# hukaixuan19970627/yolov5_obb

Measured on AMD Instinct MI355X. Metric: val.py img/s (hot path: non_max_suppression_obb, bs16) + NMS ms/img @100k cand, DOTAv1.5 1024^2, 1/2/4/8 GPU, higher is better.
Workload: dtype f16; 1 GPU; DOTAv1.5 1024^2 bs16 (BASELINE metric; configs[1] thresholds): yolov5 OBB head output (16,64512,201) fp16, 4 distinct tensors rotated (cold: 1.66 GB working set) -> non_max_suppression_obb (conf .25, iou .45, multi_label, max_det 1500), val.py --task speed hot path = dt[2] of val.py; global_batch=16, anchors_per_image=64512, nc=16, detections_per_batch=3734, parallelism=dp1 (images sharded, no data-path collective)

## Files before the change

include/obb_hip.h:

```cpp
#ifndef OBB_HIP_H
#define OBB_HIP_H

#include <stddef.h>
#include <stdint.h>

#ifdef __cplusplus
extern "C" {
#endif

#define OBB_OK 0
#define OBB_ERR_BAD_ARG (-1)
#define OBB_ERR_WORKSPACE (-2)
#define OBB_ERR_LAUNCH (-3)
#define OBB_ERR_INTERNAL (-4)
#define OBB_ERR_NO_DEVICE (-5)

#define OBB_NMS_DROP_SMALL 1

const char* obb_version(void);
int obb_device_info(int* cu_count, int* wave_size, char* arch_name, int arch_name_len);
int obb_nms_set_max_grid(int max_workgroups);

#define OBB_PROF_STAGES 8
int obb_profile_enable(int on);
int obb_profile_collect(double* ms_sum_host, int64_t* count_host, int n_stages);



size_t obb_nms_workspace_bytes(int64_t n, int64_t nseg, int kind);

int obb_nms_rotated_f32(const float* dets5, const float* scores, int64_t n, float iou_thr, int flags, int64_t max_keep,
                        int64_t* keep_out, int64_t* num_keep, void* ws, size_t ws_bytes, void* stream);

int obb_nms_rotated_f64(const double* dets5, const double* scores, int64_t n, float iou_thr, int flags, int64_t max_keep,
                        int64_t* keep_out, int64_t* num_keep, void* ws, size_t ws_bytes, void* stream);

int obb_nms_poly_f32(const float* polys, int64_t row_stride, int64_t n, float iou_thr, int64_t max_keep, int64_t* keep_out,
                     int64_t* num_keep, void* ws, size_t ws_bytes, void* stream);

int obb_merge_nms_poly_f64(const double* dets9, int64_t n, const int32_t* order, const int32_t* seg_off, int64_t nseg,
                           double thresh, int64_t* keep_out, int64_t* num_keep, void* ws, size_t ws_bytes, void* stream);

int obb_merge_nms_poly_all_f64(const double* dets9, int64_t n, const int32_t* order, const int32_t* seg_off, int64_t nseg,
                               double thresh, int64_t* keep_out, int64_t* num_keep, void* ws, size_t ws_bytes, void* stream);
// ... 131 lines not shown
```

yolov5_obb_amd/_lib.py:

```python
import ctypes as C
import os
import threading

import torch

_HERE = os.path.dirname(os.path.abspath(__file__))
LIB_PATH = os.environ.get("OBB_HIP_LIB") or os.path.join(_HERE, "libobb_hip.so")

OBB_OK = 0
OBB_NMS_DROP_SMALL = 1
_ERR = {-1: "bad argument", -2: "workspace missing or too small", -3: "kernel launch failed",
        -4: "internal error", -5: "no usable HIP device"}

_lib = None
_lock = threading.RLock()

_vp, _i64, _i32, _f32, _sz = C.c_void_p, C.c_int64, C.c_int, C.c_float, C.c_size_t

SIGNATURES = {
    "obb_version": (C.c_char_p, []),
    "obb_device_info": (_i32, [C.POINTER(_i32), C.POINTER(_i32), C.c_char_p, _i32]),
    "obb_nms_set_max_grid": (_i32, [_i32]),
    "obb_profile_enable": (_i32, [_i32]),
    "obb_profile_collect": (_i32, [_vp, _vp, _i32]),
    "obb_nms_workspace_bytes": (_sz, [_i64, _i64, _i32]),
    "obb_nms_rotated_f32": (_i32, [_vp, _vp, _i64, _f32, _i32, _i64, _vp, _vp, _vp, _sz, _vp]),
    "obb_nms_rotated_f64": (_i32, [_vp, _vp, _i64, _f32, _i32, _i64, _vp, _vp, _vp, _sz, _vp]),
    "obb_nms_poly_f32": (_i32, [_vp, _i64, _i64, _f32, _i64, _vp, _vp, _vp, _sz, _vp]),
    "obb_merge_nms_poly_f64": (_i32, [_vp, _i64, _vp, _vp, _i64, C.c_double, _vp, _vp, _vp, _sz, _vp]),
    "obb_merge_nms_poly_all_f64": (_i32, [_vp, _i64, _vp, _vp, _i64, C.c_double, _vp, _vp, _vp, _sz, _vp]),
    "obb_merge_nms_hbb_f64": (_i32, [_vp, _i64, _i64, _vp, _vp, _i64, C.c_double, _vp, _vp, _vp, _sz, _vp]),
    "obb_task1_parse_tiles": (_i64, [_vp, _i64, _i64, _vp, _vp, _vp, _vp, _vp, _vp]),
    "obb_task1_format_rows": (_i64, [_vp, _vp, _vp, _vp, _vp, _i64, _vp, _i64]),
    "obb_task1_parse_dets": (_i64, [_vp, _i64, _i64, _vp, _vp, _vp, _vp]),
    "obb_task1_parse_gt": (_i64, [_vp, _i64, _i64, _vp, _vp, _vp, _vp]),
    "obb_eval_best_gt_f64": (_i32, [_vp, _vp, _i64, _vp, _vp, _i64, _vp, _vp, _vp]),
    "obb_nms_obb_workspace_bytes": (_sz, [_i64, _i64, _i64, _i32]),
    "obb_non_max_suppression_obb": (_i32, [_vp, _i32, _i64, _i64, _i64, _f32, _f32, _vp, _i32, _i32, _i32, _i64, _i64, _f32,
                                           _vp, _i64, _i64, _i64, _vp, _i32, _vp, _vp, _vp, _sz, _vp]),
    "obb_non_max_suppression_obb_col": (_i32, [_vp, _vp, _i32, _i64, _i64, _i64, _f32, _f32, _vp, _i32, _i32, _i32, _i64, _i64, _f32,
                                               _vp, _i64, _i64, _i64, _vp, _i32, _vp, _vp, _vp, _sz, _vp]),
    "obb_nms_obb_state_bytes": (_sz, [_i64]),
    "obb_non_max_suppression_obb_st": (_i32, [_vp, _vp, _i32, _i64, _i64, _i64, _f32, _f32, _vp, _i32, _i32, _i32, _i64, _i64, _f32,
                                              _vp, _i64, _i64, _i64, _vp, _i32, _vp, _vp, _vp, _sz, _vp, _sz, _vp]),
    "obb_non_max_suppression_obb_head": (_i32, [_i32, _vp, _i32, _i64, _i64, _i64, _vp, _vp, _vp, _vp, _f32, _f32, _vp, _i32, _i32, _i32,
# ... 214 lines not shown
```

yolov5_obb_amd/csrc/nms.hip:

```cpp
#include <hip/hip_runtime.h>
#include <cstring>
#include <stdint.h>
#include <stdlib.h>
#include <stdio.h>
#include <string.h>
#include <hip/hip_fp16.h>
#include "launch_once.h"
#include "obb_device.h"
#include "nms_core.h"
#include "nms_mk.h"
#include "obb_hip.h"
#include "psrs_sort.h"
#include "nms_small.h"
#include "segsort.h"

namespace obb {

enum { PROF_DECODE = 0, PROF_SEGSORT, PROF_PREP, PROF_STEPS, PROF_GATHER, PROF_NMS_SORT, PROF_NMS_PREP, PROF_NMS_STEPS, PROF_N };
struct ProfState {
  int on = 0;
  static constexpr int kMax = 8192;
  hipEvent_t ev0[kMax], ev1[kMax];
  int id[kMax];
  int created = 0, used = 0;
// ... 1032 lines not shown
    const int want = 2048 < ProfState::kMax ? 2048 : ProfState::kMax;
    while (g_prof.created < want) {
      if (hipEventCreate(&g_prof.ev0[g_prof.created]) != hipSuccess) return OBB_ERR_INTERNAL;
      if (hipEventCreate(&g_prof.ev1[g_prof.created]) != hipSuccess) { hipEventDestroy(g_prof.ev0[g_prof.created]); return OBB_ERR_INTERNAL; }
      g_prof.created++;
    }
  }
  return OBB_OK;
}

int obb_profile_collect(double* ms_sum, int64_t* count, int n_stages) {
  for (int i = 0; i < n_stages; i++) { ms_sum[i] = 0.0; count[i] = 0; }
  for (int k = 0; k < g_prof.used; k++) {
    float ms = 0.f;
    if (hipEventSynchronize(g_prof.ev1[k]) != hipSuccess) return OBB_ERR_INTERNAL;
    if (hipEventElapsedTime(&ms, g_prof.ev0[k], g_prof.ev1[k]) != hipSuccess) return OBB_ERR_INTERNAL;
    const int id = g_prof.id[k];
    if (id < n_stages) { ms_sum[id] += ms; count[id]++; }
  }
  g_prof.used = 0;
  return OBB_OK;
}

int obb_nms_set_max_grid(int max_workgroups) {
  g_max_grid = max_workgroups > 0 ? max_workgroups : 0;
  return OBB_OK;
}

const char* obb_version(void) { return "obb_hip 0.2 (gfx950)"; }

int obb_device_info(int* cu_count, int* wave_size, char* arch_name, int arch_name_len) {
  int dev = 0;
  if (hipGetDevice(&dev) != hipSuccess) return OBB_ERR_NO_DEVICE;
  hipDeviceProp_t p;
  if (hipGetDeviceProperties(&p, dev) != hipSuccess) return OBB_ERR_NO_DEVICE;
  if (cu_count) *cu_count = p.multiProcessorCount;
  if (wave_size) *wave_size = p.warpSize;
  if (arch_name && arch_name_len > 0) { strncpy(arch_name, p.gcnArchName, arch_name_len - 1); arch_name[arch_name_len - 1] = 0; }
  return OBB_OK;
}

}

#ifdef OBB_SMALL_TRACE
extern "C" int obb_debug_small_trace2(unsigned long long* words) {
  static unsigned long long zero2[2048 * 8];
  if (hipDeviceSynchronize() != hipSuccess) return -1;
  if (hipMemcpyFromSymbol(words, HIP_SYMBOL(obb::g_small_trace2), sizeof(obb::g_small_trace2)) != hipSuccess) return -1;
  return hipMemcpyToSymbol(HIP_SYMBOL(obb::g_small_trace2), zero2, sizeof(obb::g_small_trace2)) == hipSuccess ? 0 : -1;
}
extern "C" int obb_debug_small_trace(unsigned long long* seg_words, unsigned long long* tail_words) {
  if (hipDeviceSynchronize() != hipSuccess) return -1;
  if (hipMemcpyFromSymbol(seg_words, HIP_SYMBOL(obb::g_small_trace), sizeof(obb::g_small_trace)) != hipSuccess) return -2;
  if (hipMemcpyFromSymbol(tail_words, HIP_SYMBOL(obb::g_small_trace_tail), sizeof(obb::g_small_trace_tail)) != hipSuccess) return -3;
  static unsigned long long zero[2048 * 16];
  if (hipMemcpyToSymbol(HIP_SYMBOL(obb::g_small_trace), zero, sizeof(obb::g_small_trace)) != hipSuccess) return -4;
  if (hipMemcpyToSymbol(HIP_SYMBOL(obb::g_small_trace_tail), zero, sizeof(obb::g_small_trace_tail)) != hipSuccess) return -5;
  return 0;
}
#endif
```

yolov5_obb_amd/csrc/nms_small.h:

```cpp
#pragma once

namespace obb {

#ifdef OBB_SMALL_TRACE
__device__ unsigned long long g_small_trace[2048 * 16];
__device__ unsigned long long g_small_trace_tail[2048 * 4];
__device__ unsigned long long g_small_trace2[2048 * 8];
#define STRACE(kind, ...) do { if (threadIdx.x == 0 && blockIdx.x < 2048) { const unsigned long long v_[] = {__VA_ARGS__}; unsigned long long* o_ = g_small_trace + blockIdx.x * 16; o_[0] = (kind); for (int z_ = 0; z_ < (int)(sizeof(v_) / 8) && z_ < 15; z_++) o_[1 + z_] = v_[z_]; } } while (0)
#endif
constexpr int kSmallMax = OBB_NMS_SMALL_SEG;
constexpr int kSmallWords = kSmallMax / 64;
constexpr int kSmallThreads = 512;
constexpr int kSmallWaves = kSmallThreads / 64;

struct SmallArgs {
  const float4* rec;
  const u64* alive;
  const int* seg_begin;
  const int* seg_end;
  int* keep_cnt;
  int64_t* keep_out;
  int* too_big;
  float thr;
  int max_keep;
  const unsigned long long* keys_sorted;
  const uint32_t* vals_sorted;
  const int* mode;
  int ncs;
  unsigned long long* pub_key;
  uint32_t* pub_val;
  long long n_pos;
  int helpers;
  const int* help_cnt;
  const int* work;
  const int* seg_np;
  int* seg_ticket;
  u64* part_main;
  u64* part_help;
  const unsigned long long* keys_in;
  const float4* cand;
  const int* cnt;
  const int* tiny;
  long long cap_img, max_nms, A;
  int nc;
  float class_offset;
  int* seg_max;
};
struct SmallFromSort { static constexpr bool kSelf = false; };
constexpr int kSmallClipWaves = 4;
constexpr int kSmallSplit1 = 128;
constexpr int kSmallHelpMax = 256;
__host__ __device__ __forceinline__ int small_parts(int n) {
  return n <= kSmallSplit1 ? 1 : (n <= 192 ? 2 : (n <= 256 ? 4 : (n <= 320 ? 6 : 8)));
}
struct SmallNoTail {
  struct Args {};
  static __device__ __forceinline__ void run(const SmallArgs&, const Args&, unsigned char*, int) {}
};

template <class G>
__device__ __attribute__((noinline)) int small_quick(const float4* ra, const float4* rb, float thr) {
  return G::classify_quick(ra, rb, thr, true);
}

template <class G>
__device__ __attribute__((noinline)) uint32_t small_slice_bits(const float4* s_rec, int i0, int n, uint32_t arow16, float4 cq, int j, bool jv) {
  const int lane = threadIdx.x & 63;
  const int ir = i0 + (lane & 15);
  const float4 rq = s_rec[(ir < n ? ir : 0) * G::RECQ];
// ... 4 lines not shown
    const float dx = cq.x - a.x, dy = cq.y - a.y;
    const float rs = a.z + cq.z;
    const float d2 = dx * dx + dy * dy;
    const bool apart = (d2 > rs * rs) & (fminf(a.w, cq.w) >= 2.34e-9f * d2);
    const bool row_ok = ((arow16 >> r) & 1u) != 0u && i0 + r < n;
    const bool pass = !apart & jv & (j > i0 + r) & row_ok;
    bits |= pass ? (1u << r) : 0u;
  }
  return bits;
}

template <class G>
struct SmallWave {
  float scr[G::SCR * 64];
  uint32_t q0[128], q1[128], q2[128];
};

template <class G, class FRONT>
__device__ __forceinline__ int small_segment(const SmallArgs& a, unsigned char* s_raw) {
  __shared__ int s_next, s_nkept, s_qcnt[kSmallWaves], s_qhead[kSmallWaves], s_qcnt2[kSmallWaves], s_last;
  __shared__ uint32_t s_kept[kSmallMax];
  __shared__ unsigned long long s_pk[kSmallMax];
  __shared__ uint32_t s_pv[kSmallMax];
  float4* s_rec = reinterpret_cast<float4*>(s_raw);
  u64* s_mask = reinterpret_cast<u64*>(s_rec + (size_t)kSmallMax * G::RECQ);
  u64* s_alive = s_mask + (size_t)kSmallMax * kSmallWords;
  SmallWave<G>* s_wave = reinterpret_cast<SmallWave<G>*>(s_alive + 8);
  const int tid = threadIdx.x, lane = tid & 63, wv = tid >> 6;
  int seg = (int)blockIdx.x - a.helpers, part = 0, np = 1, hbase = 0;
  if (seg < 0) {
    const int h = (int)blockIdx.x;
    if (h >= *a.help_cnt) {
#ifdef OBB_SMALL_TRACE
      STRACE(1ull, (unsigned long long)wall_clock64());
#endif
      return -1;
    }
    const int e = a.work[h];
    if (e < 0) return -1;
    seg = e & 0xffffff; part = e >> 24;
  }
  if (a.helpers > 0) { const int v = a.seg_np[seg]; if ((v & 255) > 1) { np = v & 255; hbase = v >> 8; } }
#ifdef OBB_SMALL_TRACE
  unsigned long long tt[8]; int ti_ = 0, nd0 = 0, nd1 = 0, nd2 = 0, nit = 0;
  unsigned long long acc_d0 = 0, acc_d1 = 0, acc_d2 = 0, acc_draw = 0, acc_l0 = 0, acc_l1 = 0, acc_l2 = 0;
#define SSTAMP() do { tt[ti_++] = wall_clock64(); } while (0)
// ... 11 lines not shown
      if (tid == 0) { stg_agent(a.keep_cnt + seg, 0); if (n > kSmallMax) atomicMax(a.too_big, n); }
      return seg;
    }
  } else {
    sb = a.seg_begin[seg]; n = a.seg_end[seg] - sb;
    if (n <= 0) return part == 0 ? seg : -1;
    if (n > kSmallMax) { if (tid == 0 && part == 0) atomicMax(a.too_big, n); return part == 0 ? seg : -1; }
  }
  const bool pub = a.pub_key != nullptr;
  if constexpr (!FRONT::kSelf) {
    for (int t = tid; t < n * G::RECQ; t += kSmallThreads) s_rec[t] = a.rec[(size_t)sb * G::RECQ + t];
    for (int t = tid; t < n * kSmallWords; t += kSmallThreads) s_mask[t] = 0ull;
    if (pub)
      for (int t = tid; t < n; t += kSmallThreads) { s_pk[t] = a.keys_sorted[(size_t)sb + t]; s_pv[t] = a.vals_sorted[(size_t)sb + t]; }
    if (tid < kSmallWords) {
      const int w0 = (sb >> 6) + tid, sh = sb & 63;
      u64 v = a.alive[w0] >> sh;
      if (sh) v |= a.alive[w0 + 1] << (64 - sh);
      const int left = n - tid * 64;
      if (left <= 0) v = 0ull; else if (left < 64) v &= (1ull << left) - 1ull;
      s_alive[tid] = v;
    }
  }
  if (tid == 0) s_next = 0;
  __syncthreads();
  SSTAMP();
  const float thr = a.thr;
  SmallWave<G>& W = s_wave[wv];
  PairQueue Q0{W.q0, 0, 0}, Q1{W.q1, 0, 0}, Q2{W.q2, 0, 0};
  auto hit = [&](bool h, int i, int j) { if (h) atomicOr(&s_mask[i * kSmallWords + (j >> 6)], 1ull << (j & 63)); };
  auto drain2 = [&](int cnt) {
#ifdef OBB_SMALL_TRACE
    nd2++;
#endif
    wave_sync();
    bool h = false;
    int i = 0, j = 0;
    if (lane < cnt) {
      const uint32_t e = W.q2[(Q2.head + lane) & 127];
      i = (int)(e >> 16); j = (int)(e & 0xffffu);
      h = nms_stage_exact<G>(s_rec + i * G::RECQ, s_rec + j * G::RECQ, thr, W.scr + lane);
    }
    hit(h, i, j);
    Q2.head = (Q2.head + cnt) & 127; Q2.count -= cnt;
    wave_sync();
  };
  auto drain1 = [&](int cnt) {
#ifdef OBB_SMALL_TRACE
    nd1++;
#endif
    wave_sync();
    int res = 0, i = 0, j = 0;
    uint32_t e = 0;
// ... 1 lines not shown
      e = W.q1[(Q1.head + lane) & 127];
      i = (int)(e >> 16); j = (int)(e & 0xffffu);
      res = nms_stage_full<G>(s_rec + i * G::RECQ, s_rec + j * G::RECQ, thr);
    }
    hit(res == 1, i, j);
    Q1.head = (Q1.head + cnt) & 127; Q1.count -= cnt;
    Q2.push(res == 2, e);
    wave_sync();
    if (Q2.count >= 64) drain2(64);
  };
  auto drain0 = [&](int cnt) {
#ifdef OBB_SMALL_TRACE
    nd0++;
#endif
    wave_sync();
    int res = 0, i = 0, j = 0;
    uint32_t e = 0;
    if (lane < cnt) {
      e = W.q0[(Q0.head + lane) & 127];
      i = (int)(e >> 16); j = (int)(e & 0xffffu);
      res = small_quick<G>(s_rec + i * G::RECQ, s_rec + j * G::RECQ, thr);
    }
    hit(res == 1, i, j);
    Q0.head = (Q0.head + cnt) & 127; Q0.count -= cnt;
    Q1.push(res == 3, e);
    Q2.push(res == 2, e);
    wave_sync();
    if (Q2.count >= 64) drain2(64);
    if (Q1.count >= 64) drain1(64);
  };
  {
    const int nb = (n + 63) >> 6;
    const int nitems = nb * (nb + 1) / 2 * 4;
    for (;;) {
      int it = 0;
#ifdef OBB_SMALL_TRACE
      const unsigned long long tdr_ = wall_clock64();
#endif
      if (lane == 0) it = atomicAdd(&s_next, 1);
      it = __builtin_amdgcn_readfirstlane(it) * np + part;
#ifdef OBB_SMALL_TRACE
      acc_draw += wall_clock64() - tdr_;
#endif
      if (it >= nitems) break;
#ifdef OBB_SMALL_TRACE
      nit++;
#endif
      const int tile = it >> 2, quarter = it & 3;
      int ti = 0, rem = tile;
      while (rem >= nb - ti) { rem -= nb - ti; ti++; }
      const int tj = ti + rem;
      const int j = tj * 64 + lane;
      const bool jv = j < n && ((s_alive[tj] >> lane) & 1ull);
      const float4 cq = s_rec[(j < n ? j : 0) * G::RECQ];
      const int i0 = ti * 64 + quarter * 16;
      const uint32_t arow16 = (uint32_t)(s_alive[ti] >> (quarter * 16)) & 0xffffu;
      if (i0 >= n || arow16 == 0u) continue;
      uint32_t bits = small_slice_bits<G>(s_rec, i0, n, arow16, cq, j, jv);
      while (__ballot(bits != 0u)) {
        const bool has = bits != 0u;
        const int r = __builtin_ctz(bits | 0x10000u);
        Q0.push(has, ((uint32_t)(i0 + r) << 16) | (uint32_t)j);
        bits &= bits - 1u;
#ifdef OBB_SMALL_TRACE
        if (Q0.count >= 64) { const unsigned long long td_ = wall_clock64(); drain0(64); acc_d0 += wall_clock64() - td_; }
#else
        if (Q0.count >= 64) drain0(64);
#endif
      }
    }
    SSTAMP();
    for (int stage = 0; stage < 3; stage++) {
      PairQueue& Q = stage == 0 ? Q0 : (stage == 1 ? Q1 : Q2);
#ifdef OBB_SMALL_TRACE
      const unsigned long long tl_ = wall_clock64();
      struct LeftT { unsigned long long& a; unsigned long long t; __device__ ~LeftT() { a += wall_clock64() - t; } } lt_{stage == 0 ? acc_l0 : (stage == 1 ? acc_l1 : acc_l2), tl_};
#endif
      for (;;) {
        if (stage <= 1 && Q2.count > 64) drain2(64);
        if (stage == 0 && Q1.count > 64) drain1(64);
        if (lane == 0) { s_qcnt[wv] = Q.count; s_qhead[wv] = Q.head; if (stage == 1) s_qcnt2[wv] = Q2.count; }
        __syncthreads();
        if (stage == 1) {
          int t12 = 0, fit = 1;
#pragma unroll
          for (int w = 0; w < kSmallWaves; w++) { t12 += s_qcnt[w] + s_qcnt2[w]; fit &= (s_qcnt[w] + s_qcnt2[w] <= 128) ? 1 : 0; }
#ifdef OBB_SMALL_TRACE
          { int t1_ = 0; for (int w = 0; w < kSmallWaves; w++) t1_ += s_qcnt[w]; if (tid == 0 && blockIdx.x < 2048 && g_small_trace2[blockIdx.x * 8 + 7] == 0ull) g_small_trace2[blockIdx.x * 8 + 7] = 1ull + (unsigned long long)t1_ + ((unsigned long long)(t12 - t1_) << 20); }
#endif
          if (t12 <= 64 * kSmallClipWaves && fit) {
            while (Q1.count > 0) {
              wave_sync();
              const int c1 = Q1.count < 64 ? Q1.count : 64;
              const bool mv = lane < c1;
              const uint32_t e1 = mv ? W.q1[(Q1.head + lane) & 127] : 0u;
// ... 9 lines not shown
        pre[0] = 0;
#pragma unroll
        for (int w = 0; w < kSmallWaves; w++) pre[w + 1] = pre[w] + s_qcnt[w];
        const int total = pre[kSmallWaves];
        if (total == 0) { __syncthreads(); break; }
        const int g = wv * 64 + lane;
        int res = 0, i = 0, j = 0;
        uint32_t e = 0;
        const bool busy = wv * 64 < total;
        if (busy && g < total) {
          int w = 0;
#pragma unroll
          for (int u = 1; u < kSmallWaves; u++) w += (g >= pre[u]) ? 1 : 0;
          const uint32_t* ring = stage == 0 ? s_wave[w].q0 : (stage == 1 ? s_wave[w].q1 : s_wave[w].q2);
          e = ring[(s_qhead[w] + (g - pre[w])) & 127];
          i = (int)(e >> 16); j = (int)(e & 0xffffu);
          const float4* ra = s_rec + i * G::RECQ;
          const float4* rb = s_rec + j * G::RECQ;
          if (stage == 0) res = small_quick<G>(ra, rb, thr);
          else if (stage == 1) res = nms_stage_full<G>(ra, rb, thr);
          else res = nms_stage_exact<G>(ra, rb, thr, W.scr + lane) ? 1 : 0;
        }
        hit(res == 1, i, j);
#ifdef OBB_SMALL_TRACE
        if (busy) { if (stage == 0) nd0++; else if (stage == 1) nd1++; else nd2++; }
#endif
        __syncthreads();
        {
          const int room = kSmallWaves * 64 - pre[wv];
          const int took = room <= 0 ? 0 : (room < s_qcnt[wv] ? room : s_qcnt[wv]);
          Q.head = (Q.head + took) & 127; Q.count -= took;
        }
        if (busy) {
          if (stage == 0) { Q1.push(res == 3, e); Q2.push(res == 2, e); }
          else if (stage == 1) Q2.push(res == 2, e);
          wave_sync();
        }
        __syncthreads();
      }
    }
  }
  SSTAMP();
  __syncthreads();
  if (np > 1) {
    auto part_buf = [&](int p) -> u64* {
      return p == 0 ? a.part_main + (size_t)sb * kSmallWords : a.part_help + (size_t)(hbase + p - 1) * kSmallMax * kSmallWords;
    };
    u64* mine = part_buf(part);
    for (int t = tid; t < n * kSmallWords; t += kSmallThreads) stg_agent(mine + t, s_mask[t]);
    asm volatile("s_waitcnt vmcnt(0)" ::: "memory");
    __syncthreads();
    if (tid == 0) s_last = __hip_atomic_fetch_add(a.seg_ticket + seg, 1, __ATOMIC_RELAXED, __HIP_MEMORY_SCOPE_AGENT) == np - 1 ? 1 : 0;
    __syncthreads();
    if (!s_last) {
#ifdef OBB_SMALL_TRACE
      STRACE(2ull, (unsigned long long)seg | ((unsigned long long)part << 24) | ((unsigned long long)np << 28), (unsigned long long)n, 0ull, tt[0], tt[1], tt[2], tt[3], (unsigned long long)wall_clock64(), 0ull, 0ull, (unsigned long long)nit, (unsigned long long)nd0, (unsigned long long)nd1, (unsigned long long)nd2);
#endif
      return -1;
    }
    for (int p = 0; p < np; p++) {
      if (p == part) continue;
      const u64* src = part_buf(p);
      for (int t = tid; t < n * kSmallWords; t += kSmallThreads) { const u64 v = ldg_agent(src + t); if (v) s_mask[t] |= v; }
// ... 2 lines not shown
  }
  SSTAMP();
  if (wv == 0) {
    u64 cur = lane < kSmallWords ? s_alive[lane] : 0ull;
    int k = 0;
    const int limit = a.max_keep > 0 ? a.max_keep : 0x7fffffff;
    const int nw = (n + 63) >> 6;
    for (int w = 0; w < nw && k < limit; w++) {
      u64 pending = ((u64)(uint32_t)__builtin_amdgcn_readlane((int)(cur >> 32), w) << 32) | (uint32_t)__builtin_amdgcn_readlane((int)cur, w);
      while (pending && k < limit) {
        const int b = __builtin_ctzll(pending), i = w * 64 + b;
        if (lane == 0) s_kept[k] = (uint32_t)i;
        k++;
        if (lane < kSmallWords) cur &= ~s_mask[i * kSmallWords + lane];
        pending = ((u64)(uint32_t)__builtin_amdgcn_readlane((int)(cur >> 32), w) << 32) | (uint32_t)__builtin_amdgcn_readlane((int)cur, w);
        pending = b < 63 ? (pending & (~0ull << (b + 1))) : 0ull;
      }
    }
    if (lane == 0) s_nkept = k;
  }
  __syncthreads();
  SSTAMP();
  const int nk = s_nkept;
  if (pub) {
    const int md = FRONT::kSelf ? md_self : a.mode[seg / a.ncs];
    for (int k = tid; k < nk; k += kSmallThreads) {
      const int i = (int)s_kept[k];
      const unsigned long long key = s_pk[i];
      stg_agent(a.pub_key + (size_t)sb + k, md == 1 ? ((key << 8) | (key >> 56)) : key);
      stg_agent(a.pub_val + (size_t)sb + k, s_pv[i]);
    }
    if (tid == 0) stg_agent(a.keep_cnt + seg, nk);
  } else {
    for (int k = tid; k < nk; k += kSmallThreads) a.keep_out[(size_t)sb + k] = (int64_t)(sb + (int)s_kept[k]);
    if (tid == 0) a.keep_cnt[seg] = nk;
  }
#ifdef OBB_SMALL_TRACE
  SSTAMP();
  STRACE(3ull, (unsigned long long)seg | ((unsigned long long)part << 24) | ((unsigned long long)np << 28), (unsigned long long)n, (unsigned long long)nk, tt[0], tt[1], tt[2], tt[3], tt[4], tt[5], tt[6], (unsigned long long)nit, (unsigned long long)nd0, (unsigned long long)nd1, (unsigned long long)nd2);
  if (tid == 0 && blockIdx.x < 2048) { unsigned long long* o_ = g_small_trace2 + blockIdx.x * 8; o_[0] = acc_d0; o_[1] = acc_d1; o_[2] = acc_d2; o_[3] = acc_draw; o_[4] = acc_l0; o_[5] = acc_l1; o_[6] = acc_l2; }
#endif
#undef SSTAMP
  return seg;
}

template <class G, class TAIL, class FRONT = SmallFromSort>
__global__ __launch_bounds__(kSmallThreads) void k_nms_small(SmallArgs a, typename TAIL::Args ta) {
  extern __shared__ __attribute__((aligned(16))) unsigned char s_raw[];
  const int seg = small_segment<G, FRONT>(a, s_raw);
  if (seg < 0) return;
  TAIL::run(a, ta, s_raw, seg);
}

static_assert((size_t)kSmallMax * RotGeom::RECQ * 16 + (size_t)kSmallMax * kSmallWords * 8 + 64 + sizeof(SmallWave<RotGeom>) * kSmallWaves +
              kSmallMax * 4 + kSmallMax * 12 + 256 <= 160 * 1024, "k_nms_small: LDS budget");
static_assert(kSmallMax % 64 == 0 && kSmallMax <= 65535, "k_nms_small: pair entries are (i << 16 | j)");

template <class G>
static size_t small_lds_bytes() {
  return (size_t)kSmallMax * G::RECQ * 16 + (size_t)kSmallMax * kSmallWords * 8 + 8 * 8 + sizeof(SmallWave<G>) * kSmallWaves;
}

}
```

yolov5_obb_amd/csrc/nmsobb_impl.h:

```cpp
#pragma once
#include "dtype_device.h"
#include "obb_device.h"
#include "segsort.h"

namespace obb {

struct ClassMask { unsigned long long w[4]; int all; };

template <typename T> __device__ __forceinline__ float mul_in_dtype(float a, float b);
template <> __device__ __forceinline__ float mul_in_dtype<float>(float a, float b) { return a * b; }
template <> __device__ __forceinline__ float mul_in_dtype<__half>(float a, float b) { return __half2float(__float2half_rn(a * b)); }
template <typename T> __device__ __forceinline__ float thr_in_dtype(float t);
template <> __device__ __forceinline__ float thr_in_dtype<float>(float t) { return t; }
template <> __device__ __forceinline__ float thr_in_dtype<__half>(float t) { return __half2float(__float2half_rn(t)); }

__device__ __forceinline__ unsigned long long argmax_key(float v, int i) {
  const uint32_t b = __float_as_uint(v + 0.0f);
  const uint32_t m = (v != v) ? 0xFFFFFFFFu : (b & 0x80000000u) ? ~b : (b | 0x80000000u);
  return ((unsigned long long)m << 32) | (unsigned long long)(0xFFFFFFFFu - (uint32_t)i);
}
template <int CTRL>
__device__ __forceinline__ unsigned long long dpp_max_u64(unsigned long long k) {
  const uint32_t lo = (uint32_t)__builtin_amdgcn_update_dpp(0, (int)(uint32_t)k, CTRL, 0xF, 0xF, true);
  const uint32_t hi = (uint32_t)__builtin_amdgcn_update_dpp(0, (int)(uint32_t)(k >> 32), CTRL, 0xF, 0xF, true);
// ... 1135 lines not shown

static int obb_carve(void* base, int64_t bs, int64_t cap_img, int64_t ncs, ObbCarve* cv) {
  cap_img = round_cap(cap_img);
  size_t off = 0;
  auto take = [&](size_t bytes) { size_t o = off; off += align_up(bytes); return base ? (char*)base + o : (char*)nullptr; };
  const size_t n = (size_t)bs * cap_img;
  cv->cand = (float4*)take(n * 32);
  cv->keys_a = (unsigned long long*)take(n * 8); cv->keys_b = (unsigned long long*)take(n * 8);
  cv->vals_a = (uint32_t*)take(n * 4); cv->vals_b = (uint32_t*)take(n * 4);
  cv->cnt = (int*)take(bs * 4 * kCntPad); cv->sort_begin = (int*)take(bs * 4); cv->sort_end = (int*)take(bs * 4);
  cv->img_end = (int*)take(bs * 4); cv->mode = (int*)take(bs * 4); cv->tiny = (int*)take(bs * 4);
  cv->ticket = (int*)take(64 + (size_t)(bs + 1) * 4);
  cv->seg_size = (int*)take((size_t)bs * 256 * 4);
  cv->srs_hist = (uint32_t*)take((size_t)bs * ((size_t)(cap_img + kSrsTile - 1) / kSrsTile) * 256 * 4);
  cv->keep = (int64_t*)take(n * 8);
  cv->nms_base = base ? (char*)base + off : nullptr;
  int rc = carve(cv->nms_base, (int64_t)n, bs * ncs, RotGeom::RECQ, cap_max(bs * ncs), &cv->nms);
  if (rc) return rc;
  off += cv->nms.total;
  cv->total = off;
  return OBB_OK;
}

struct HeadFront;
static int launch_decode_head(const HeadFront& h, const DecodeArgs& d, int dtype, hipStream_t st);

static int run_nms_obb(const void* pred, const void* objcol, int dtype, int64_t bs, int64_t A, int64_t no, float conf_thres, float iou_thres,
                       const int32_t* classes_host, int n_classes, int agnostic, int multi_label, int64_t max_det, int64_t max_nms,
                       float max_wh, const float* extra8, int64_t n_extra, int64_t cap_img, int64_t expected_cand, float* out,
                       int out_packed, int64_t* out_count, int64_t* status, void* ws, size_t ws_bytes, hipStream_t st, void* state = nullptr,
                       size_t state_bytes = 0, const HeadFront* head = nullptr) {
  const int nc = (int)(no - 5 - 180);
  if (bs < 1 || A < 1 || nc < 1 || nc > 256 || max_det < 1 || cap_img < 1 || (!pred && !head) || !out || !out_count || !status)
    return OBB_ERR_BAD_ARG;
  if (A * nc + n_extra > 0xffffffffLL || bs * cap_img > 0x7fffffffLL) return OBB_ERR_BAD_ARG;
  if (dtype != 0 && dtype != 1) return OBB_ERR_BAD_ARG;
  const int64_t seg_hint = (expected_cand >> 32) & 0x1fffffff;
  const bool small_hint = ((expected_cand >> 62) & 1) != 0;
  expected_cand &= 0xffffffffll;
  cap_img = round_cap(cap_img);
  const int ncs = agnostic ? 1 : nc;
  const int class_ok = (!agnostic && nc > 1 && A + n_extra < (1ll << 24) && iou_thres >= 0.f && max_wh > 0.f) ? 1 : 0;
  ObbCarve cv;
  int rc = obb_carve(ws, bs, cap_img, ncs, &cv);
  if (rc) return rc;
  if (!ws || ws_bytes < cv.total) return OBB_ERR_WORKSPACE;
// ... 33 lines not shown
  }
  d.rows_per_thread = (bs * A >= 4LL * kDecThreads * 480) ? 4 : (bs * A >= 2LL * kDecThreads * 480) ? 2 : 1;
  dim3 gd((unsigned)((A + kDecThreads * d.rows_per_thread - 1) / (kDecThreads * d.rows_per_thread)), (unsigned)bs);
  {
    ProfScope ps(PROF_DECODE, st);
    if (head) {
      rc = launch_decode_head(*head, d, dtype, st);
      if (rc) return rc;
    } else if (dtype == 0) k_decode<float><<<gd, kDecThreads, 0, st>>>(d);
    else k_decode<__half><<<gd, kDecThreads, 0, st>>>(d);
  }
  if (n_extra > 0 && extra8) k_append_extra<<<(unsigned)((n_extra + 255) / 256), 256, 0, st>>>(extra8, (int)n_extra, A, nc, d);
  if (small_hint && class_ok)
    k_tiny_cross<<<dim3(kTinyParts, (unsigned)bs), 256, 0, st>>>(cv.cand, cv.keys_a, cv.cnt, cap_img, max_wh, iou_thres, cv.tiny);
  const unsigned gs = (unsigned)((bs + 255) / 256);
  Carve& nv = cv.nms;
  const int64_t max_seg = (max_nms > 0 && max_nms < cap_img) ? max_nms : cap_img;
  const int nms_capmax = cap_max(bs * ncs);
  const int plan_chunk = kCapFirst < nms_capmax ? kCapFirst : nms_capmax;
  const bool small_nms = lds_sort && class_ok && seg_hint > 0 && seg_hint <= kSmallMax && iou_thres >= 0.f && bs * ncs <= 65535;
  const int plan_nb = (bs * ncs > 1 && !small_nms) ? nms_grid(bs * ncs, bs * max_seg, kCapFirst) : 0;
  const int helpers_env = [] { const char* e = getenv("OBB_NMS_SMALL_HELPERS"); const int v = (e && *e) ? atoi(e) : -1; return v > kSmallHelpMax ? kSmallHelpMax : v; }();
  const int self_env = [] { const char* e = getenv("OBB_NMS_SELF_SORT"); return (e && *e >= '0' && *e <= '2') ? *e - '0' : 2; }();
  const bool self_possible = small_nms && !out_packed && (int64_t)ncs * kSmallMax <= cap_img && self_env != 0;
  int helpers = 0;
  if (small_nms && !(self_possible && self_env == 2 && helpers_env < 0)) {
    const int64_t free_cus = (int64_t)hw_cu_count() - bs * ncs;
    helpers = helpers_env >= 0 ? helpers_env : (int)(free_cus < 0 ? 0 : (free_cus > kSmallHelpMax ? kSmallHelpMax : free_cus));
  }
  int *help_work = nullptr, *seg_np = nullptr, *seg_ticket = nullptr;
  u64 *part_main = nullptr, *part_help = nullptr;
  if (helpers > 0) {
    const size_t nseg_b = align_up((size_t)(bs * ncs) * 4), work_b = align_up((size_t)helpers * 4);
    const size_t main_b = align_up((size_t)bs * cap_img * kSmallWords * 8), help_b = align_up((size_t)helpers * kSmallMax * kSmallWords * 8);
    const size_t have = (size_t)((bs * ncs < (int64_t)cu_count()) ? bs * ncs : (int64_t)cu_count()) * (size_t)nv.ecap * 4;
    if (work_b + 2 * nseg_b + main_b + help_b > have) helpers = 0;
    else {
      char* p = reinterpret_cast<char*>(nv.edges);
      help_work = (int*)p; p += work_b;
      seg_np = (int*)p; p += nseg_b;
      seg_ticket = (int*)p; p += nseg_b;
      part_main = (u64*)p; p += main_b;
      part_help = (u64*)p;
    }
  }
  const bool self_sort = self_possible && helpers == 0;
// ... 60 lines not shown
  a.rec = nv.rec; a.order = nullptr; a.alive = nv.alive; a.seg_begin = nv.seg_begin; a.seg_end = nv.seg_end;
  a.keep_cnt = nv.keep_cnt; a.keep_out = cv.keep;
  a.rows = nv.rows; a.nrows = nv.nrows; a.edges = nv.edges; a.nedges = nv.nedges;
  a.ecap = nv.ecap; a.n = (int)(bs * cap_img); a.capmax = cap_max(bs * ncs);
  a.max_keep = (int)max_det; a.window = nms_window(max_det); a.thr = iou_thres; a.cull = (iou_thres >= 0.f) ? 1 : 0;
  const bool fused_out = small_nms && !out_packed;
  if (small_nms) {
    ProfScope ps(PROF_STEPS, st);
    static OncePerDevice attr;
    const size_t lds = small_lds_bytes<RotGeom>();
    if (const int attr_dev = attr.need(); attr_dev != OncePerDevice::kDone) {
      if (hipFuncSetAttribute((const void*)k_nms_small<RotGeom, SmallNoTail>, hipFuncAttributeMaxDynamicSharedMemorySize, (int)lds) != hipSuccess ||
          hipFuncSetAttribute((const void*)k_nms_small<RotGeom, SmallGather>, hipFuncAttributeMaxDynamicSharedMemorySize, (int)lds) != hipSuccess ||
          hipFuncSetAttribute((const void*)k_nms_small<RotGeom, SmallGather, SmallSelfSort>, hipFuncAttributeMaxDynamicSharedMemorySize, (int)lds) != hipSuccess)
        return OBB_ERR_LAUNCH;
      attr.mark(attr_dev);
    }
    SmallArgs sa{};
    sa.rec = nv.rec; sa.alive = nv.alive; sa.seg_begin = nv.seg_begin; sa.seg_end = nv.seg_end; sa.keep_cnt = nv.keep_cnt;
    sa.keep_out = cv.keep; sa.too_big = cv.ticket + 8; sa.thr = iou_thres; sa.max_keep = (int)max_det;
    sa.ncs = ncs; sa.mode = cv.mode;
    sa.helpers = helpers; sa.help_cnt = cv.ticket + 12; sa.work = help_work; sa.seg_np = seg_np; sa.seg_ticket = seg_ticket;
    sa.part_main = part_main; sa.part_help = part_help;
    const unsigned gsmall = (unsigned)(bs * ncs + helpers);
    if (fused_out) {
      sa.keys_sorted = cv.keys_b; sa.vals_sorted = cv.vals_b; sa.pub_key = cv.keys_a; sa.pub_val = cv.vals_a; sa.n_pos = bs * cap_img;
      SmallGather::Args ga{};
      ga.cand = cv.cand; ga.cnt = cv.cnt; ga.tiny = cv.tiny; ga.info = cv.ticket; ga.ticket = cv.ticket + 16;
      ga.out = out; ga.out_count = out_count; ga.status = status; ga.cap_img = cap_img; ga.max_det = max_det; ga.bs = (int)bs;
      ga.clean_cnt = kept ? cv.cnt : nullptr; ga.clean_tiny = kept ? cv.tiny : nullptr;
      if (self_sort) {
        sa.pub_key = cv.keys_b; sa.pub_val = cv.vals_b; sa.keys_sorted = nullptr; sa.vals_sorted = nullptr;
        sa.keys_in = cv.keys_a; sa.cand = cv.cand; sa.cnt = cv.cnt; sa.tiny = cv.tiny; sa.cap_img = cap_img; sa.max_nms = max_nms; sa.A = A; sa.nc = nc;
        sa.class_offset = max_wh; sa.seg_max = cv.ticket + 4;
        k_nms_small<RotGeom, SmallGather, SmallSelfSort><<<gsmall, kSmallThreads, lds, st>>>(sa, ga);
      } else
      k_nms_small<RotGeom, SmallGather><<<gsmall, kSmallThreads, lds, st>>>(sa, ga);
    } else {
      k_nms_small<RotGeom, SmallNoTail><<<gsmall, kSmallThreads, lds, st>>>(sa, SmallNoTail::Args{});
    }
  } else {
    ProfScope ps(PROF_STEPS, st);
    rc = nms_steps(0, a, nv, bs * ncs, bs * max_seg, st, kNmsBarZeroed | ((lds_sort && plan_nb > 0) ? kNmsPlanned : 0));
    if (rc) return rc;
  }
  if (!fused_out) {
// ... 11 lines not shown
```

yolov5_obb_amd/utils/general.py:

```python
import ctypes as C
import threading
import time

import torch

from .. import _lib
from ..lazy import LazyTensor

pi = 3.141592

_MAX_WH = 4096
_PENDING = -(1 << 62)
_POLL_SECONDS = 2e-3
_POLL_GIVE_UP = 1.0
_MAX_NMS = 30000
_CSL = 180
_cap_memo = {}
_ws_memo = {}
_meta_memo = {}
_cand_memo = {}
_SORT_LDS_HINT = 6144
_SORT_LDS_MAX = 8192
_hold = {}
_HOLD = 8
# ... 27 lines not shown
    idx = torch.cuda.current_device() if idx is None else idx
    ext = _lib.compiled()
    if ext is not None:
        return ext.hint_get(idx, int(A), int(nc), bool(multi_label), float(conf_thres))
    key = _key(idx, A, nc, multi_label, conf_thres)
    if key not in _cand_memo and key not in _seg_memo:
        return None
    return {"cand": _cand_memo.get(key, _SORT_LDS_HINT), "seg": _seg_memo.get(key, 1), "cap": _cap_memo.get(key, 0),
            "small_boxes": bool(_small_memo.get(key, False)), "small_resolved": bool(_small_memo.get((key, "resolved"), False))}


def hint_set(device, A, nc, multi_label, conf_thres, cand=None, seg=None):
    idx = torch.device(device).index
    idx = torch.cuda.current_device() if idx is None else idx
    ext = _lib.compiled()
    if ext is not None:
        ext.hint_set(idx, int(A), int(nc), bool(multi_label), float(conf_thres), -1 if cand is None else int(cand), -1 if seg is None else int(seg))
        return
    key = _key(idx, A, nc, multi_label, conf_thres)
    if cand is not None:
        _cand_memo[key] = int(cand); _hold[key, "cand"] = 0
    if seg is not None:
        _seg_memo[key] = int(seg); _hold[key, "seg"] = 0


def _label_rows(labels, bs, nc, device):
    rows = []
    theta0 = torch.tensor((0 - 90) / 180, dtype=torch.float32).mul(pi).item()
    for b in range(bs):
        if b < len(labels) and len(labels[b]):
            lb = labels[b].to(device=device, dtype=torch.float32)
            r = torch.zeros((lb.shape[0], 8), device=device, dtype=torch.float32)
            r[:, 0] = b
            r[:, 1:5] = lb[:, 1:5]
            r[:, 5] = theta0
            r[:, 6] = 1.0
            r[:, 7] = lb[:, 0].long().float()
            rows.append(r)
    return torch.cat(rows, 0).contiguous() if rows else None


def _objectness_column(prediction, pred):
    tag = getattr(prediction, "_obb_objcol", None)
    if tag is None or pred is not prediction:
        return None
    col, version = tag
# ... 167 lines not shown
```

Before: 142,000 img/s.

## Add early diagonal-tile pruning pass to small-segment rotated NMS kernel

Adds a first pass to the small NMS kernel that evaluates only the first 64-row diagonal tile's pairs and records which pairs are still undecided. A wave-level greedy scan then resolves definitely-kept and definitely-suppressed boxes in that tile and clears suppressed boxes from the alive mask. Queued expensive pairs whose endpoints are already dead are dropped before the full pass runs. The aim is to skip exact polygon IoU work for boxes that top-scoring boxes already suppress. In exchange it adds an extra LDS buffer, an extra round with barriers, and per-block atomic counters with a host readback API. It is on by default through an environment threshold.

```diff
diff --git a/include/obb_hip.h b/include/obb_hip.h
--- a/include/obb_hip.h
+++ b/include/obb_hip.h
@@ -20,6 +20,7 @@
 const char* obb_version(void);
 int obb_device_info(int* cu_count, int* wave_size, char* arch_name, int arch_name_len);
 int obb_nms_set_max_grid(int max_workgroups);
+int obb_nms_small_prune_counters(int64_t* counters2_host);
 
 #define OBB_PROF_STAGES 8
 int obb_profile_enable(int on);
diff --git a/yolov5_obb_amd/_lib.py b/yolov5_obb_amd/_lib.py
--- a/yolov5_obb_amd/_lib.py
+++ b/yolov5_obb_amd/_lib.py
@@ -21,6 +21,7 @@
     "obb_version": (C.c_char_p, []),
     "obb_device_info": (_i32, [C.POINTER(_i32), C.POINTER(_i32), C.c_char_p, _i32]),
     "obb_nms_set_max_grid": (_i32, [_i32]),
+    "obb_nms_small_prune_counters": (_i32, [_vp]),
     "obb_profile_enable": (_i32, [_i32]),
     "obb_profile_collect": (_i32, [_vp, _vp, _i32]),
     "obb_nms_workspace_bytes": (_sz, [_i64, _i64, _i32]),
diff --git a/yolov5_obb_amd/csrc/nms.hip b/yolov5_obb_amd/csrc/nms.hip
--- a/yolov5_obb_amd/csrc/nms.hip
+++ b/yolov5_obb_amd/csrc/nms.hip
@@ -1078,6 +1078,21 @@
   return OBB_OK;
 }
 
+int obb_nms_small_prune_counters(int64_t* counters2) {
+  if (!counters2) return OBB_ERR_BAD_ARG;
+  counters2[0] = counters2[1] = 0;
+  const PruneLast& pl = g_prune_last;
+  if (!pl.ptr) return OBB_OK;
+  int cur = 0, w[2] = {0, 0};
+  if (hipGetDevice(&cur) != hipSuccess) return OBB_ERR_NO_DEVICE;
+  if (cur != pl.dev && hipSetDevice(pl.dev) != hipSuccess) return OBB_ERR_NO_DEVICE;
+  const bool ok = hipMemcpyAsync(w, pl.ptr, sizeof(w), hipMemcpyDeviceToHost, pl.st) == hipSuccess && hipStreamSynchronize(pl.st) == hipSuccess;
+  if (cur != pl.dev) hipSetDevice(cur);
+  if (!ok) return OBB_ERR_INTERNAL;
+  counters2[0] = w[0]; counters2[1] = w[1];
+  return OBB_OK;
+}
+
 int obb_nms_set_max_grid(int max_workgroups) {
   g_max_grid = max_workgroups > 0 ? max_workgroups : 0;
   return OBB_OK;
@@ -1105,6 +1120,12 @@
   if (hipMemcpyFromSymbol(words, HIP_SYMBOL(obb::g_small_trace2), sizeof(obb::g_small_trace2)) != hipSuccess) return -1;
   return hipMemcpyToSymbol(HIP_SYMBOL(obb::g_small_trace2), zero2, sizeof(obb::g_small_trace2)) == hipSuccess ? 0 : -1;
 }
+extern "C" int obb_debug_small_trace3(unsigned long long* words) {
+  static unsigned long long zero3[2048 * 8];
+  if (hipDeviceSynchronize() != hipSuccess) return -1;
+  if (hipMemcpyFromSymbol(words, HIP_SYMBOL(obb::g_small_trace3), sizeof(obb::g_small_trace3)) != hipSuccess) return -1;
+  return hipMemcpyToSymbol(HIP_SYMBOL(obb::g_small_trace3), zero3, sizeof(obb::g_small_trace3)) == hipSuccess ? 0 : -1;
+}
 extern "C" int obb_debug_small_trace(unsigned long long* seg_words, unsigned long long* tail_words) {
   if (hipDeviceSynchronize() != hipSuccess) return -1;
   if (hipMemcpyFromSymbol(seg_words, HIP_SYMBOL(obb::g_small_trace), sizeof(obb::g_small_trace)) != hipSuccess) return -2;
diff --git a/yolov5_obb_amd/csrc/nms_small.h b/yolov5_obb_amd/csrc/nms_small.h
--- a/yolov5_obb_amd/csrc/nms_small.h
+++ b/yolov5_obb_amd/csrc/nms_small.h
@@ -1,4 +1,5 @@
 #pragma once
+#include "prune_status.h"
 
 namespace obb {
 
@@ -6,6 +7,7 @@
 __device__ unsigned long long g_small_trace[2048 * 16];
 __device__ unsigned long long g_small_trace_tail[2048 * 4];
 __device__ unsigned long long g_small_trace2[2048 * 8];
+__device__ unsigned long long g_small_trace3[2048 * 8];
 #define STRACE(kind, ...) do { if (threadIdx.x == 0 && blockIdx.x < 2048) { const unsigned long long v_[] = {__VA_ARGS__}; unsigned long long* o_ = g_small_trace + blockIdx.x * 16; o_[0] = (kind); for (int z_ = 0; z_ < (int)(sizeof(v_) / 8) && z_ < 15; z_++) o_[1 + z_] = v_[z_]; } } while (0)
 #endif
 constexpr int kSmallMax = OBB_NMS_SMALL_SEG;
@@ -45,6 +47,8 @@
   int nc;
   float class_offset;
   int* seg_max;
+  int prune_min;
+  unsigned long long* prune_cnt;
 };
 struct SmallFromSort { static constexpr bool kSelf = false; };
 constexpr int kSmallClipWaves = 4;
@@ -95,6 +99,7 @@
   __shared__ uint32_t s_kept[kSmallMax];
   __shared__ unsigned long long s_pk[kSmallMax];
   __shared__ uint32_t s_pv[kSmallMax];
+  __shared__ u64 s_und[kPruneTile * kSmallWords];
   float4* s_rec = reinterpret_cast<float4*>(s_raw);
   u64* s_mask = reinterpret_cast<u64*>(s_rec + (size_t)kSmallMax * G::RECQ);
   u64* s_alive = s_mask + (size_t)kSmallMax * kSmallWords;
@@ -152,6 +157,8 @@
       s_alive[tid] = v;
     }
   }
+  const bool prune = a.prune_min > 0 && np == 1 && n > a.prune_min && n > kPruneTile;
+  if (prune) for (int t = tid; t < kPruneTile * kSmallWords; t += kSmallThreads) s_und[t] = 0ull;
   if (tid == 0) s_next = 0;
   __syncthreads();
   SSTAMP();
@@ -159,6 +166,9 @@
   SmallWave<G>& W = s_wave[wv];
   PairQueue Q0{W.q0, 0, 0}, Q1{W.q1, 0, 0}, Q2{W.q2, 0, 0};
   auto hit = [&](bool h, int i, int j) { if (h) atomicOr(&s_mask[i * kSmallWords + (j >> 6)], 1ull << (j & 63)); };
+  bool mark = prune;
+  int prune_cleared = -1;
+  auto undecided = [&](int res, int i, int j) { if (mark && res >= 2) atomicOr(&s_und[i * kSmallWords + (j >> 6)], 1ull << (j & 63)); };
   auto drain2 = [&](int cnt) {
 #ifdef OBB_SMALL_TRACE
     nd2++;
@@ -206,6 +216,7 @@
       res = small_quick<G>(s_rec + i * G::RECQ, s_rec + j * G::RECQ, thr);
     }
     hit(res == 1, i, j);
+    undecided(res, i, j);
     Q0.head = (Q0.head + cnt) & 127; Q0.count -= cnt;
     Q1.push(res == 3, e);
     Q2.push(res == 2, e);
@@ -213,9 +224,11 @@
     if (Q2.count >= 64) drain2(64);
     if (Q1.count >= 64) drain1(64);
   };
-  {
-    const int nb = (n + 63) >> 6;
-    const int nitems = nb * (nb + 1) / 2 * 4;
+  const int nb = (n + 63) >> 6;
+  const int nitems = nb * (nb + 1) / 2 * 4;
+  for (int round = 0, nrounds = prune ? 2 : 1; round < nrounds; round++) {
+    const int lim = mark ? nb * 4 : nitems;
+    const int nstages = mark ? 0 : 3;
     for (;;) {
       int it = 0;
 #ifdef OBB_SMALL_TRACE
@@ -226,7 +239,7 @@
 #ifdef OBB_SMALL_TRACE
       acc_draw += wall_clock64() - tdr_;
 #endif
-      if (it >= nitems) break;
+      if (it >= lim) break;
 #ifdef OBB_SMALL_TRACE
       nit++;
 #endif
@@ -253,8 +266,12 @@
 #endif
       }
     }
-    SSTAMP();
-    for (int stage = 0; stage < 3; stage++) {
+    if (!mark) SSTAMP();
+    else {
+      if (Q0.count > 0) drain0(Q0.count);
+      __syncthreads();
+    }
+    for (int stage = 0; stage < nstages; stage++) {
       PairQueue& Q = stage == 0 ? Q0 : (stage == 1 ? Q1 : Q2);
 #ifdef OBB_SMALL_TRACE
       const unsigned long long tl_ = wall_clock64();
@@ -310,6 +327,7 @@
           else res = nms_stage_exact<G>(ra, rb, thr, W.scr + lane) ? 1 : 0;
         }
         hit(res == 1, i, j);
+        if (stage == 0) undecided(res, i, j);
 #ifdef OBB_SMALL_TRACE
         if (busy) { if (stage == 0) nd0++; else if (stage == 1) nd1++; else nd2++; }
 #endif
@@ -327,6 +345,73 @@
         __syncthreads();
       }
     }
+    if (!mark) break;
+    mark = false;
+#ifdef OBB_SMALL_TRACE
+    const unsigned long long tp1_ = wall_clock64(); unsigned long long tp2_ = 0ull; int p_cleared_ = 0, p_ku_ = 0;
+#endif
+    if (wv == 0) {
+      const u64 al0v = s_alive[0];
+      const u64 al0 = ((u64)(uint32_t)__builtin_amdgcn_readfirstlane((int)(al0v >> 32)) << 32) | (uint32_t)__builtin_amdgcn_readfirstlane((int)al0v);
+      const int before = lane < nb ? __popcll(s_alive[lane]) : 0;
+      struct DiagRow {
+        u64 h, u;
+        __device__ __forceinline__ void operator()(int b, uint64_t& hv, uint64_t& uv) const {
+          hv = ((u64)(uint32_t)__builtin_amdgcn_readlane((int)(h >> 32), b) << 32) | (uint32_t)__builtin_amdgcn_readlane((int)h, b);
+          uv = ((u64)(uint32_t)__builtin_amdgcn_readlane((int)(u >> 32), b) << 32) | (uint32_t)__builtin_amdgcn_readlane((int)u, b);
+        }
+      };
+      uint64_t kept0, unk0;
+      const u64 dead0 = prune_tile(al0, DiagRow{s_mask[lane * kSmallWords], s_und[lane * kSmallWords]}, &kept0, &unk0);
+      if ((kept0 >> lane) & 1ull)
+        for (int w = 1; w < nb; w++) { const u64 hv = s_mask[lane * kSmallWords + w]; if (hv) atomicAnd(&s_alive[w], ~hv); }
+      if (lane == 0) s_alive[0] = al0 & ~dead0;
+      wave_sync();
+      int cleared = lane < nb ? before - __popcll(s_alive[lane]) : 0;
+#pragma unroll
+      for (int d = 1; d < 8; d <<= 1) cleared += __shfl_xor(cleared, d);
+      prune_cleared = cleared;
+#ifdef OBB_SMALL_TRACE
+      p_cleared_ = cleared; p_ku_ = __popcll(kept0) | (__popcll(unk0) << 8);
+#endif
+    }
+    if (tid == 0) s_next = nb * 4;
+    __syncthreads();
+#ifdef OBB_SMALL_TRACE
+    tp2_ = wall_clock64();
+#endif
+    int dropped = 0;
+    for (int ring = 1; ring <= 2; ring++) {
+      PairQueue& Q = ring == 1 ? Q1 : Q2;
+      uint32_t* q = ring == 1 ? W.q1 : W.q2;
+      for (int left = Q.count; left > 0; left -= 64) {
+        wave_sync();
+        const int c = left < 64 ? left : 64;
+        uint32_t e = 0u;
+        bool keep = false;
+        if (lane < c) {
+          e = q[(Q.head + lane) & 127];
+          const int i = (int)(e >> 16), j = (int)(e & 0xffffu);
+          keep = ((s_alive[i >> 6] >> (i & 63)) & (s_alive[j >> 6] >> (j & 63)) & 1ull) != 0ull;
+        }
+        Q.head = (Q.head + c) & 127; Q.count -= c;
+        dropped += c;
+        const int had = Q.count;
+        Q.push(keep, e);
+        dropped -= Q.count - had;
+        wave_sync();
+      }
+    }
+    if (Q2.count > 64) drain2(64);
+    if (Q1.count > 64) drain1(64);
+#ifdef OBB_SMALL_TRACE
+    if (tid == 0 && blockIdx.x < 2048) {
+      unsigned long long* o_ = g_small_trace3 + blockIdx.x * 8;
+      o_[0] = 1ull + (unsigned long long)n; o_[1] = tp1_; o_[2] = tp2_; o_[3] = wall_clock64(); o_[4] = (unsigned long long)p_cleared_;
+      o_[5] = (unsigned long long)dropped; o_[6] = (unsigned long long)p_ku_;
+    }
+#endif
+    (void)dropped;
   }
   SSTAMP();
   __syncthreads();
@@ -375,6 +460,7 @@
   __syncthreads();
   SSTAMP();
   const int nk = s_nkept;
+  if (tid == 0 && prune_cleared >= 0) atomicAdd(a.prune_cnt, 1ull | ((unsigned long long)prune_cleared << 32));
   if (pub) {
     const int md = FRONT::kSelf ? md_self : a.mode[seg / a.ncs];
     for (int k = tid; k < nk; k += kSmallThreads) {
@@ -406,7 +492,7 @@
 }
 
 static_assert((size_t)kSmallMax * RotGeom::RECQ * 16 + (size_t)kSmallMax * kSmallWords * 8 + 64 + sizeof(SmallWave<RotGeom>) * kSmallWaves +
-              kSmallMax * 4 + kSmallMax * 12 + 256 <= 160 * 1024, "k_nms_small: LDS budget");
+              kSmallMax * 4 + kSmallMax * 12 + kPruneTile * kSmallWords * 8 + 256 <= 160 * 1024, "k_nms_small: LDS budget");
 static_assert(kSmallMax % 64 == 0 && kSmallMax <= 65535, "k_nms_small: pair entries are (i << 16 | j)");
 
 template <class G>
diff --git a/yolov5_obb_amd/csrc/nmsobb_impl.h b/yolov5_obb_amd/csrc/nmsobb_impl.h
--- a/yolov5_obb_amd/csrc/nmsobb_impl.h
+++ b/yolov5_obb_amd/csrc/nmsobb_impl.h
@@ -1181,6 +1181,10 @@
   return OBB_OK;
 }
 
+struct PruneLast { const int* ptr; hipStream_t st; int dev; };
+static thread_local PruneLast g_prune_last = {nullptr, nullptr, 0};
+constexpr int kSmallPruneMin = 128;
+
 struct HeadFront;
 static int launch_decode_head(const HeadFront& h, const DecodeArgs& d, int dtype, hipStream_t st);
 
@@ -1260,6 +1264,8 @@
   const int plan_nb = (bs * ncs > 1 && !small_nms) ? nms_grid(bs * ncs, bs * max_seg, kCapFirst) : 0;
   const int helpers_env = [] { const char* e = getenv("OBB_NMS_SMALL_HELPERS"); const int v = (e && *e) ? atoi(e) : -1; return v > kSmallHelpMax ? kSmallHelpMax : v; }();
   const int self_env = [] { const char* e = getenv("OBB_NMS_SELF_SORT"); return (e && *e >= '0' && *e <= '2') ? *e - '0' : 2; }();
+  const int prune_min = [] { const char* e = getenv("OBB_NMS_SMALL_PRUNE"); const int v = (e && *e) ? atoi(e) : 1; return v <= 0 ? 0 : (v < kPruneTile ? kSmallPruneMin : v); }();
+  g_prune_last.ptr = nullptr;
   const bool self_possible = small_nms && !out_packed && (int64_t)ncs * kSmallMax <= cap_img && self_env != 0;
   int helpers = 0;
   if (small_nms && !(self_possible && self_env == 2 && helpers_env < 0)) {
@@ -1366,6 +1372,9 @@
     sa.ncs = ncs; sa.mode = cv.mode;
     sa.helpers = helpers; sa.help_cnt = cv.ticket + 12; sa.work = help_work; sa.seg_np = seg_np; sa.seg_ticket = seg_ticket;
     sa.part_main = part_main; sa.part_help = part_help;
+    sa.prune_min = prune_min; sa.prune_cnt = reinterpret_cast<unsigned long long*>(cv.ticket + 10);
+    g_prune_last.ptr = cv.ticket + 10; g_prune_last.st = st;
+    if (hipGetDevice(&g_prune_last.dev) != hipSuccess) g_prune_last.ptr = nullptr;
     const unsigned gsmall = (unsigned)(bs * ncs + helpers);
     if (fused_out) {
       sa.keys_sorted = cv.keys_b; sa.vals_sorted = cv.vals_b; sa.pub_key = cv.keys_a; sa.pub_val = cv.vals_a; sa.n_pos = bs * cap_img;
diff --git a/yolov5_obb_amd/csrc/prune_status.h b/yolov5_obb_amd/csrc/prune_status.h
--- /dev/null
+++ b/yolov5_obb_amd/csrc/prune_status.h
@@ -0,0 +1,51 @@
+#pragma once
+#include <stdint.h>
+#include "obb_device.h"
+
+namespace obb {
+
+constexpr int kPruneTile = 64;
+
+enum PruneStatus { kPruneSkip = 0, kPruneDead = 1, kPruneUnknown = 2, kPruneKept = 3 };
+
+OBB_HD int prune_status(uint64_t alive0, uint64_t dead0, uint64_t unk0, int b) {
+  const uint64_t m = 1ull << b;
+  if (!(alive0 & m)) return kPruneSkip;
+  if (dead0 & m) return kPruneDead;
+  return (unk0 & m) ? kPruneUnknown : kPruneKept;
+}
+
+OBB_HD void prune_fold(int status, uint64_t h, uint64_t u, uint64_t& dead, uint64_t& unk) {
+  if (status == kPruneUnknown) unk |= h | u;
+  else if (status == kPruneKept) { dead |= h; unk |= u; }
+}
+
+template <class Row>
+OBB_HD uint64_t prune_tile(uint64_t alive0, Row row, uint64_t* kept0, uint64_t* unk0) {
+  uint64_t dead = 0ull, unk = 0ull, kept = 0ull, unknown = 0ull;
+  uint64_t pending = alive0;
+  while (pending) {
+    const int b = __builtin_ctzll(pending);
+    const int st = prune_status(alive0, dead, unk, b);
+    uint64_t h, u;
+    row(b, h, u);
+    prune_fold(st, h, u, dead, unk);
+    if (st == kPruneKept) kept |= 1ull << b; else unknown |= 1ull << b;
+    pending = b < 63 ? (pending & ~dead & (~0ull << (b + 1))) : 0ull;
+  }
+  *kept0 = kept; *unk0 = unknown;
+  return dead & alive0;
+}
+
+OBB_HD void prune_scan(const uint64_t* alive, const uint64_t* h, const uint64_t* u, int stride, int nw, uint64_t* dead,
+                       uint64_t* kept0, uint64_t* unk0) {
+  dead[0] = prune_tile(alive[0], [&](int b, uint64_t& hv, uint64_t& uv) { hv = h[(size_t)b * stride]; uv = u[(size_t)b * stride]; },
+                       kept0, unk0);
+  for (int w = 1; w < nw; w++) {
+    uint64_t d = 0ull;
+    for (uint64_t k = *kept0; k; k &= k - 1) d |= h[(size_t)__builtin_ctzll(k) * stride + w];
+    dead[w] = d & alive[w];
+  }
+}
+
+}
diff --git a/yolov5_obb_amd/utils/general.py b/yolov5_obb_amd/utils/general.py
--- a/yolov5_obb_amd/utils/general.py
+++ b/yolov5_obb_amd/utils/general.py
@@ -73,6 +73,12 @@
         _cand_memo[key] = int(cand); _hold[key, "cand"] = 0
     if seg is not None:
         _seg_memo[key] = int(seg); _hold[key, "seg"] = 0
+
+
+def small_prune_counters():
+    w = (C.c_int64 * 2)()
+    _lib.check(_lib.lib().obb_nms_small_prune_counters(C.cast(w, C.c_void_p)), "obb_nms_small_prune_counters")
+    return int(w[0]), int(w[1])
 
 
 def _label_rows(labels, bs, nc, device):
```

Result: slower. 136,200 img/s (-4.1%).
